# HandBrake/HandBrake

Hardware: AMD Instinct MI355X
Metric: filtered frames/sec, 1080p YUV420p NLMeans+decomb chain (higher is better)
Workload: dtype u8 (f32 NLMeans weights, 16-bit fixed-point scaler as zimg, sharpen mix = the reference's f64 expression, as one f32 multiply where init proves that equal); 1 GPU; BASELINE configs[3]: decomb(31, EEDI2 bob) -> nlmeans medium -> cropscale lanczos 1920x1080 -> 3840x2160 -> lapsharp, 1080i YUV420P 8-bit in, inputs resident in HBM; input=1920x1080, output=3840x2160, streams_per_gpu=1, content=interlaced, stream_frames=48, stage_streams=2, parallelism=1 GPU(s) x 1 independent stream(s), device=AMD Radeon Graphics (gfx950:sramecc+:xnack-, 256 CUs)

## Files before the change

handbrake_amd/csrc/eedi2.hip:

```cpp
#include "eedi2_common.h"
#include "eedi2_vote.h"
#include "eedi2_dense.h"
#include "eedi2_engine.h"
#include "eedi2_mask_cells.h"
#include "eedi2_corner.h"

#include <atomic>
#include <algorithm>

namespace {

constexpr int PEAK = 255, NEUTRAL = 128;
constexpr int EEDI_MAX_FIELDS = EEDI_MAX_BATCH;
constexpr size_t GUARD = 32768;

__constant__ uint8_t c_limlut[33] = { 6, 6, 7, 7, 8, 8, 9, 9, 9, 10, 10, 11, 11, 12, 12, 12, 12, 12, 12, 12,
                                      12, 12, 12, 12, 12, 12, 12, 12, 12, 12, 12, 255, 255 };

constexpr int LIM_N = 33, LIM_PAD = 40;
__device__ __forceinline__ void lim_fill(uint8_t *tab, int tid)
{
    if (tid < LIM_N) tab[tid] = c_limlut[tid];
}

struct P3
{
    uint8_t *a[3];
    uint8_t *b[3];
    uint8_t *c[3];
    uint8_t *d[3];
    uint8_t *e[3];
    uint8_t *f[3];
    uint8_t *g[3];
    int pitch[3], width[3], height[3];
    size_t   fstride;
    uint32_t tffbits;
    const uint32_t *pflags;
    uint32_t pepoch;
};

struct PL { uint8_t *a, *b, *c, *d, *e, *f, *g; };
__device__ __forceinline__ PL plane_ptrs(const P3 &P, int pl, size_t off)
{
    PL q = { P.a[pl] + off, P.b[pl] + off, P.c[pl] + off, P.d[pl], P.e[pl] + off, P.f[pl] + off, P.g[pl] + off };
    if (q.d) q.d += off;
    return q;
}
#define FIELD_PLANE(P)                                                      \
    const int fld = (int)blockIdx.z / 3, pl = (int)blockIdx.z - 3 * fld;    \
    const int tff = (int)(((P).tffbits >> fld) & 1u);                       \
    const PL Q = plane_ptrs((P), pl, (size_t)fld * (P).fstride);            \
     \
     \
    const bool maskless = (P).pflags[blockIdx.z] != (P).pepoch;             \
    (void)tff; (void)maskless

__device__ __forceinline__ int hbhip_align_up_dev(int v, int a) { return (v + a - 1) / a * a; }

__device__ __forceinline__ int wave_list_slots(int *counter, unsigned n)
{
    const uint64_t b0 = __ballot(n & 1u), b1 = __ballot(n & 2u), b2 = __ballot(n & 4u);
    const int total = __popcll(b0) + 2 * __popcll(b1) + 4 * __popcll(b2);
    auto below = [](uint64_t m) { return (int)__builtin_amdgcn_mbcnt_hi((uint32_t)(m >> 32), __builtin_amdgcn_mbcnt_lo((uint32_t)m, 0u)); };
    int base = 0;
    if (total)
    {
        if ((threadIdx.x & 63) == 0) base = atomicAdd(counter, total);
        base = __builtin_amdgcn_readfirstlane(base);
    }
    return base + below(b0) + 2 * below(b1) + 4 * below(b2);
}

__device__ __forceinline__ int sad3(const uint8_t *a, int ai, const uint8_t *b, int bi)
{
    return iabs((int)a[ai - 1] - (int)b[bi - 1]) + iabs((int)a[ai] - (int)b[bi]) + iabs((int)a[ai + 1] - (int)b[bi + 1]);
}

constexpr int ABSENT = 1000;

__device__ __forceinline__ int mid9(int &v0, int &v1, int &v2, int &v3, int &v4, int &v5, int &v6, int &v7, int &v8, int n)
{
    cswap(v0, v3); cswap(v1, v7); cswap(v2, v5); cswap(v4, v8);
    cswap(v0, v7); cswap(v2, v4); cswap(v3, v8); cswap(v5, v6);
    cswap(v0, v2); cswap(v1, v3); cswap(v4, v5); cswap(v7, v8);
// ... 693 lines not shown
            act |= (uint32_t)a << j;
            inactive |= (up[j] | dn[j]) & ((2u << maxdt) - 1u);
        }
        if (__any(act != 0))
        {
            const uint32_t *tr = &s_tri[0][b];
            if (__all(inactive == 0))
                calc_dir_dense_vote<RD, false, RD, 0>(tr, maxdt, up, dn, act, nt13, nt19, &s_out[0][lx]);
            else
            {
                constexpr int RH = RD >= 8 ? RD / 2 : RD;
                calc_dir_dense_vote<RH, true, RD, 0>(tr, maxdt, up, dn, act, nt13, nt19, &s_out[0][lx]);
                if constexpr (RH < RD) calc_dir_dense_vote<RD - RH, true, RD, RH>(tr, maxdt, up, dn, act, nt13, nt19, &s_out[0][lx]);
            }
#ifdef HBHIP_DEV_STATS
            if (lane == 0) { CD_STAT(8, 1); CD_STAT(9, __all(inactive == 0)); }
#endif
        }
        __syncthreads();
    }
    else if (count)
    {
        for (int p = tid; p < count; p += CD_W)
        {
            const uint32_t id = s_list[p];
            const int j = (int)(id >> 8), lx = (int)(id & 255u), y = y0 + j, px = x0 + lx, b = lx + CD_HALO - 1;
            const int startu = max(-px + 1, -maxdt), stopu = min(width - 2 - px, maxdt);
            uint64_t pass = 0;
            if (stopu >= startu)
            {
                const int nb = stopu - startu + 1;
                pass = (nb >= 64 ? ~0ull : ((1ull << nb) - 1ull)) << (startu + maxdt);
                if (y != 1)          pass &= calc_dir_window(s_bits[j], b - maxdt, lenmask);
                if (y != height - 2) pass &= __brevll(calc_dir_window(s_bits[j + 2], b - maxdt, lenmask)) >> (64 - len);
            }
#ifdef HBHIP_DEV_STATS
            {
                int n = __popcll(pass), mx = n, sm = n, ln = 1;
                for (int o = 32; o; o >>= 1) { mx = max(mx, __shfl_xor(mx, o)); sm += __shfl_xor(sm, o); ln += __shfl_xor(ln, o); }
                const uint64_t act = __ballot(1);
                if (lane == __ffsll((unsigned long long)act) - 1) { CD_STAT(3, 1); CD_STAT(4, sm); CD_STAT(5, mx); CD_STAT(6, ln); }
            }
#endif
            const uint32_t *tr = &s_tri[j][b];
            int out;
            if (len <= 32)
                out = edge ? calc_dir_search<true, uint32_t>(tr, (uint32_t)pass, maxdt, y == 1, y == height - 2, nt13, nt19)
                           : calc_dir_search<false, uint32_t>(tr, (uint32_t)pass, maxdt, false, false, nt13, nt19);
            else
                out = edge ? calc_dir_search<true, uint64_t>(tr, pass, maxdt, y == 1, y == height - 2, nt13, nt19)
                           : calc_dir_search<false, uint64_t>(tr, pass, maxdt, false, false, nt13, nt19);
            s_out[j][lx] = (uint8_t)out;
        }
        __syncthreads();
    }
#pragma unroll
    for (int jr = 0; jr < R; jr += CD_W / 64)
    {
        const int j = jr + (tid >> 6), y = y0 + j, xb = x0 + 4 * lane;
        if (j < R && y < height && xb < pitch)
            *reinterpret_cast<uint32_t *>(Q.c + (size_t)y * pitch + xb) = pad_bytes(reinterpret_cast<const uint32_t *>(&s_out[j][0])[lane], xb, width, padv);
    }
}


__device__ __forceinline__ int dir_map_px(int u0, int u1, int u2, int c0, int c1, int c2, int n0, int n1, int n2,
                                          bool up_ok, bool dn_ok, int expand, const uint8_t *limlut)
{
    const bool h0 = up_ok && u0 != PEAK, h1 = up_ok && u1 != PEAK, h2 = up_ok && u2 != PEAK;
    const bool h3 = c0 != PEAK, h4 = !expand && c1 != PEAK, h5 = c2 != PEAK;
    const bool h6 = dn_ok && n0 != PEAK, h7 = dn_ok && n1 != PEAK, h8 = dn_ok && n2 != PEAK;
    const int u = h0 + h1 + h2 + h3 + h4 + h5 + h6 + h7 + h8;
    if (u < (expand ? 5 : 4)) return expand ? c1 : PEAK;
    int v0 = h0 ? u0 : ABSENT, v1 = h1 ? u1 : ABSENT, v2 = h2 ? u2 : ABSENT;
    int v3 = h3 ? c0 : ABSENT, v4 = h4 ? c1 : ABSENT, v5 = h5 ? c2 : ABSENT;
    int v6 = h6 ? n0 : ABSENT, v7 = h7 ? n1 : ABSENT, v8 = h8 ? n2 : ABSENT;
    int s0 = v0, s1 = v1, s2 = v2, s3 = v3, s4 = v4, s5 = v5, s6 = v6, s7 = v7, s8 = v8;
    const int mid = mid9(s0, s1, s2, s3, s4, s5, s6, s7, s8, u);
    const int lim = limlut[iabs(mid - NEUTRAL) >> 2];
    int sum = 0, count = 0;
    vote1(v0, mid, lim, sum, count); vote1(v1, mid, lim, sum, count); vote1(v2, mid, lim, sum, count);
    vote1(v3, mid, lim, sum, count); vote1(v4, mid, lim, sum, count); vote1(v5, mid, lim, sum, count);
    vote1(v6, mid, lim, sum, count); vote1(v7, mid, lim, sum, count); vote1(v8, mid, lim, sum, count);
    const int val = vote_avg(sum + mid, count + 1);
    if (expand) return count >= 5 ? (val & 0xff) : c1;
    if (count < 4 || (count < 5 && c1 == PEAK)) return PEAK;
    return val & 0xff;
}

__device__ __forceinline__ uint32_t ff_bytes(uint32_t v)
{
    return (((v & 0x7f7f7f7fu) + 0x01010101u) & v) & 0x80808080u;
}

constexpr uint32_t PK_ABSENT_HI = 0x7f00u;
__device__ __forceinline__ u16x2 limlut2(u16x2 i)
{
    const u16x2 g = pk_lt(pk1(7), i);
    const u16x2 l = __builtin_elementwise_min((u16x2)(((i - g) >> 1) + pk1(6)), pk1(12));
    const u16x2 big = pk_lt(pk1(30), i) * pk1(255);
    return __builtin_elementwise_max(l, big);
}
#define PK_BYTES(hi, lo, a, b) __builtin_amdgcn_perm((hi), (lo), 0x0c000c00u | ((uint32_t)(b) << 16) | (uint32_t)(a))

template <int K>
__device__ __forceinline__ uint32_t dir_map_pair(const Win12 &wu, const Win12 &wc, const Win12 &wd, int expand)
{
    u16x2 v[9];
    {
        const Win12 *rows[3] = { &wu, &wc, &wd };
#pragma unroll
        for (int r = 0; r < 3; r++)
        {
            const uint32_t w0 = rows[r]->w0, w1 = rows[r]->w1, w2 = rows[r]->w2;
            if (K == 0)
            {
                v[3 * r + 0] = pk(PK_BYTES(w1, w0, 3, 4));
                v[3 * r + 1] = pk(PK_BYTES(w1, w0, 4, 5));
                v[3 * r + 2] = pk(PK_BYTES(w1, w0, 5, 6));
            }
            else
            {
                v[3 * r + 0] = pk(PK_BYTES(w1, w0, 5, 6));
                v[3 * r + 1] = pk(PK_BYTES(w1, w0, 6, 7));
                v[3 * r + 2] = pk(PK_BYTES(w2, w1, 3, 4));
            }
        }
    }
    const u16x2 c1 = v[4];
    u16x2 a[9];
    uint32_t absent = 0;
#pragma unroll
    for (int i = 0; i < 9; i++)
    {
        a[i] = (u16x2)((v[i] + pk1(1)) >> 8);
        absent += un(a[i]);
        v[i] = v[i] + a[i] * pk1(PK_ABSENT_HI);
    }
    u16x2 s0 = v[0], s1 = v[1], s2 = v[2], s3 = v[3], s4 = v[4], s5 = v[5], s6 = v[6], s7 = v[7], s8 = v[8];
    cswap2(s0, s3); cswap2(s1, s7); cswap2(s2, s5); cswap2(s4, s8);
    cswap2(s0, s7); cswap2(s2, s4); cswap2(s3, s8); cswap2(s5, s6);
    cswap2(s0, s2); cswap2(s1, s3); cswap2(s4, s5); cswap2(s7, s8);
    cswap2(s1, s4); cswap2(s3, s6); cswap2(s5, s7);
    cswap2(s0, s1); cswap2(s2, s4); cswap2(s3, s5); cswap2(s6, s8);
    cswap2(s2, s3); cswap2(s4, s5); cswap2(s6, s7);
    cswap2(s1, s2); cswap2(s3, s4); cswap2(s5, s6);
    const u16x2 ab = pk(absent), one = pk1(1), zero = pk1(0);
    const uint32_t m5 = un(zero - pk_lt(pk1(3), ab));
    const uint32_t m7 = un(zero - pk_lt(one, ab));
    const uint32_t modd = un((ab & one) - one);
#define PK_SEL(m, x, y) (((m) & (x)) | (~(m) & (y)))
    const uint32_t hi = PK_SEL(m5, un(s2), PK_SEL(m7, un(s3), un(s4)));
    const uint32_t lo = PK_SEL(m5, un(s1), PK_SEL(m7, un(s2), un(s3)));
    const u16x2 mid = pk(PK_SEL(modd, hi, un((u16x2)((pk(lo) + pk(hi) + one) >> 1))));
    const i16x2 t = __builtin_bit_cast(i16x2, (u16x2)(mid - pk1(NEUTRAL)));
    const u16x2 lim1 = limlut2(__builtin_bit_cast(u16x2, __builtin_elementwise_max(t, (i16x2)(-t))) >> 2) + one;
    u16x2 sum = zero, cnt = zero;
#pragma unroll
    for (int i = 0; i < 9; i++)
    {
        const u16x2 d = __builtin_elementwise_max(v[i], mid) - __builtin_elementwise_min(v[i], mid);
        const u16x2 in = pk_lt(d, lim1);
        cnt += in;
        sum += in * v[i];
    }
    const uint32_t sm = un((u16x2)(sum + mid)), ct = un(cnt);
    uint32_t out = 0;
#pragma unroll
    for (int h = 0; h < 2; h++)
    {
        const int n = 9 - (int)((absent >> (16 * h)) & 0xffffu);
        const int count = n >= 4 ? (int)((ct >> (16 * h)) & 0xffffu) : 0;
        const int val = vote_avg((int)((sm >> (16 * h)) & 0xffffu), count + 1) & 0xff;
        const int c = (int)((un(c1) >> (16 * h)) & 0xffu);
        int res;
        if (expand) res = count >= 5 ? val : c;
        else        res = (count < 4 || (count < 5 && c == PEAK)) ? PEAK : val;
        out |= (uint32_t)res << (16 * h);
    }
#undef PK_SEL
    return out;
}

__global__ __launch_bounds__(256) void k_dir_map4(P3 P, int step, int expand)
{
    FIELD_PLANE(P);
    const int x = 4 * (blockIdx.x * blockDim.x + threadIdx.x);
    const int r = blockIdx.y * blockDim.y + threadIdx.y;
    const int pitch = P.pitch[pl], width = P.width[pl], height = P.height[pl];
    const int y0 = step == 1 ? 1 : 2 - tff;
    const int y = step == 1 ? r : 2 * r + (y0 & 1);
    if (x >= width) return;
    if (maskless)
    {
        const int ya = step == 1 ? r : 2 * r, nrows = step == 1 ? 1 : 2;
        const int out[4] = { PEAK, PEAK, PEAK, PEAK };
        for (int i = 0; i < nrows && ya + i < height; i++)
        {
            const size_t at = (size_t)(ya + i) * pitch + x;
            st4(Q.c + at, out, x, width);
            if (Q.d) st4(Q.d + at, out, x, width);
        }
        return;
    }
    const int yc = 2 * r + 1 - (y0 & 1);
    const bool copy = step != 1 && yc < height;
    uint32_t vcopy = 0;
    if (copy) vcopy = *reinterpret_cast<const uint32_t *>(Q.b + (size_t)yc * pitch + x);
    auto put_copy = [&]() {
        if (!copy) return;
        int out[4] = { (int)(vcopy & 0xff), (int)((vcopy >> 8) & 0xff), (int)((vcopy >> 16) & 0xff), (int)(vcopy >> 24) };
        st4(Q.c + (size_t)yc * pitch + x, out, x, width);
        if (Q.d) st4(Q.d + (size_t)yc * pitch + x, out, x, width);
    };
    if (y >= height) { put_copy(); return; }
    const uint8_t *dc = Q.b + (size_t)y * pitch + x;
    uint8_t *o = Q.c + (size_t)y * pitch + x;
    const bool row_ok = step == 1 ? (y >= 1 && y < height - 1) : (y >= y0 && y < height - 1);
    if (!row_ok)
    {
        const uint32_t v = *reinterpret_cast<const uint32_t *>(dc);
        int out[4] = { (int)(v & 0xff), (int)((v >> 8) & 0xff), (int)((v >> 16) & 0xff), (int)(v >> 24) };
        st4(o, out, x, width);
        if (Q.d) st4(Q.d + (size_t)y * pitch + x, out, x, width);
        put_copy();
        return;
    }
    const uint32_t own = *reinterpret_cast<const uint32_t *>(dc);
    const uint8_t *mk = Q.a + (size_t)y * pitch + x;
    const uint32_t m0 = *reinterpret_cast<const uint32_t *>(step == 1 ? mk : mk - (ptrdiff_t)pitch);
    const uint32_t m1 = step == 1 ? 0u : *reinterpret_cast<const uint32_t *>(mk + pitch);
    const bool up_ok = step == 1 || y > 1, dn_ok = step == 1 || y < height - 2;
    uint32_t work = ((ff_bytes(m0) | ff_bytes(m1)) >> 7) & bytes_in(x, 1, width - 1);
    if (expand) work &= ff_bytes(own) >> 7;
    uint32_t res = own;
    if (work)
    {
        asm volatile("" ::: "memory");
        const Win12 wc = ldwin(dc), wu = ldwin(dc - (ptrdiff_t)step * pitch), wd = ldwin(dc + (ptrdiff_t)step * pitch);
        const Win12 none = { 0xffffffffu, 0xffffffffu, 0xffffffffu };
        const Win12 eu = up_ok ? wu : none, ed = dn_ok ? wd : none;
        const uint32_t p01 = dir_map_pair<0>(eu, wc, ed, expand), p23 = dir_map_pair<2>(eu, wc, ed, expand);
        const uint32_t votes = __builtin_amdgcn_perm(p23, p01, 0x06040200u);
        const uint32_t sel = work * 255u;
        res = (res & ~sel) | (votes & sel);
    }
    int out[4] = { (int)(res & 0xff), (int)((res >> 8) & 0xff), (int)((res >> 16) & 0xff), (int)(res >> 24) };
    st4(o, out, x, width);
    if (Q.d)
    {
        int in[4] = { (int)(own & 0xff), (int)((own >> 8) & 0xff), (int)((own >> 16) & 0xff), (int)(own >> 24) };
        st4(Q.d + (size_t)y * pitch + x, in, x, width);
    }
    put_copy();
}

__device__ __forceinline__ uint32_t live3(const Win12 &w, uint32_t &centre)
{
    const uint32_t n0 = (~ff_bytes(w.w0) >> 7) & 0x01010101u, n1 = (~ff_bytes(w.w1) >> 7) & 0x01010101u, n2 = (~ff_bytes(w.w2) >> 7) & 0x01010101u;
    centre = n1;
    return __builtin_amdgcn_alignbyte(n1, n0, 3) + n1 + __builtin_amdgcn_alignbyte(n2, n1, 1);
}

#ifndef DC_THREAD_ROWS
#define DC_THREAD_ROWS 4
#endif
constexpr int DC_R = DC_THREAD_ROWS, DC_ROWS = 4 * DC_R;
__global__ __launch_bounds__(256) void k_dir_map_c(P3 P, int step, int expand, int post)
{
    __shared__ __attribute__((aligned(16))) uint8_t s_out[DC_ROWS][256];
    __shared__ uint16_t s_list[DC_ROWS * 256];
    __shared__ int s_count;
    __shared__ uint8_t s_lim[LIM_PAD];
    FIELD_PLANE(P);
    const int y0 = step == 1 ? 1 : 2 - tff;
    const int rb = blockIdx.y * DC_ROWS;
    const int bx0 = 4 * (blockIdx.x * 64), x = bx0 + 4 * threadIdx.x;
    const int yb = step == 1 ? rb : 2 * rb + (y0 & 1);
    const int pitch = P.pitch[pl], width = P.width[pl], height = P.height[pl];
    if (bx0 >= width || (step == 1 ? rb : 2 * rb) >= height) return;
    if (maskless)
    {
        if (x < width)
        {
            const int out[4] = { PEAK, PEAK, PEAK, PEAK };
#pragma unroll
            for (int h = 0; h < DC_R; h++)
            {
                const int r = rb + (int)threadIdx.y + 4 * h, ya = step == 1 ? r : 2 * r, nrows = step == 1 ? 1 : 2;
                for (int i = 0; i < nrows && ya + i < height; i++)
                {
                    const size_t at = (size_t)(ya + i) * pitch + x;
                    st4(Q.c + at, out, x, width);
                    if (Q.d) st4(Q.d + at, out, x, width);
                }
            }
        }
        return;
    }
    const int tid = threadIdx.y * 64 + threadIdx.x;
    if (tid == 0) s_count = 0;
    lim_fill(s_lim, tid);
    __syncthreads();
    uint32_t vcopy[DC_R], own[DC_R], m0[DC_R], m1[DC_R], cand[DC_R];
#pragma unroll
    for (int h = 0; h < DC_R; h++)
    {
        const int lr = (int)threadIdx.y + 4 * h, r = rb + lr, y = step == 1 ? r : 2 * r + (y0 & 1);
        const int yc = 2 * r + 1 - (y0 & 1);
        vcopy[h] = 0; own[h] = 0; m0[h] = 0; m1[h] = 0;
        if (step != 1 && x < width && yc < height) vcopy[h] = *reinterpret_cast<const uint32_t *>(Q.b + (size_t)yc * pitch + x);
        const bool inside = x < width && y < height;
        const bool row_ok = step == 1 ? (y >= 1 && y < height - 1) : (y >= y0 && y < height - 1);
        if (inside)
        {
            own[h] = *reinterpret_cast<const uint32_t *>(Q.b + (size_t)y * pitch + x);
            if (row_ok)
            {
                const uint8_t *mk = Q.a + (size_t)y * pitch + x;
                m0[h] = *reinterpret_cast<const uint32_t *>(step == 1 ? mk : mk - (ptrdiff_t)pitch);
                if (step != 1) m1[h] = *reinterpret_cast<const uint32_t *>(mk + pitch);
            }
        }
    }
    Win12 wc[DC_R], wu[DC_R], wd[DC_R];
#pragma unroll
    for (int h = 0; h < DC_R; h++)
// ... 119 lines not shown
    {
        const Win12 none = { 0xffffffffu, 0xffffffffu, 0xffffffffu };
        const Win12 wc = { s_f[lr + 1][tx], own, s_f[lr + 1][tx + 2] };
        const Win12 wu = up_ok ? Win12{ s_f[lr][tx], s_f[lr][tx + 1], s_f[lr][tx + 2] } : none;
        const Win12 wd = dn_ok ? Win12{ s_f[lr + 2][tx], s_f[lr + 2][tx + 1], s_f[lr + 2][tx + 2] } : none;
        uint32_t nc, nu, nd;
        const uint32_t s3c = live3(wc, nc), s3u = live3(wu, nu), s3d = live3(wd, nd);
        const uint32_t u = s3c - nc + s3u + s3d;
        const uint32_t enough = ((u + (uint32_t)(0x80 - 5) * 0x01010101u) >> 7) & 0x01010101u;
        const uint32_t sortpx = cand & enough;
        if (sortpx)
        {
            int at = atomicAdd(s_count, __popc(sortpx));
#pragma unroll
            for (int k = 0; k < 4; k++)
                if ((sortpx >> (8 * k)) & 1u) s_list[at++] = (uint16_t)((lr << 8) | (4 * tx + k));
        }
        (void)nu; (void)nd;
    }
    *reinterpret_cast<uint32_t *>(&s_out[lr][4 * tx]) = own;
}

template <int STEP, bool POST>
__global__ __launch_bounds__(256) void k_dir_map_fe(P3 P, uint32_t padv)
{
    __shared__ uint32_t s_f[FE_R + 2][FE_LW];
    __shared__ __attribute__((aligned(16))) uint8_t s_out[FE_R][256];
    __shared__ uint16_t s_list[FE_R * 256];
    __shared__ int s_count;
    __shared__ uint8_t s_lim[LIM_PAD];
    FIELD_PLANE(P);
    const int y0 = STEP == 1 ? 1 : 2 - tff, par = STEP == 1 ? 0 : (y0 & 1);
    const int rb = blockIdx.y * FE_R;
    const int bx0 = 256 * blockIdx.x, x = bx0 + 4 * threadIdx.x;
    const int pitch = P.pitch[pl], width = P.width[pl], height = P.height[pl];
    if (bx0 >= pitch || STEP * rb >= height) return;
    auto row_ok = [&](int y) { return STEP == 1 ? (y >= 1 && y < height - 1) : (y >= y0 && y < height - 1); };
    if (maskless)
    {
        if (x < pitch)
            for (int lr = threadIdx.y; lr < FE_R; lr += 4)
#pragma unroll
                for (int i = 0; i < STEP; i++)
                    if (STEP * (rb + lr) + i < height)
                    {
                        const size_t at = (size_t)(STEP * (rb + lr) + i) * pitch + x;
                        *reinterpret_cast<uint32_t *>(Q.c + at) = pad_bytes(0xffffffffu, x, width, padv);
                        if (POST && x < width) { const int out[4] = { PEAK, PEAK, PEAK, PEAK }; st4(Q.d + at, out, x, width); }
                    }
        return;
    }
    const int tid = threadIdx.y * 64 + threadIdx.x;
    if (tid == 0) s_count = 0;
    lim_fill(s_lim, tid);
    constexpr int NCOPY = STEP == 1 ? 1 : (FE_R + 3) / 4;
    uint32_t vcopy[NCOPY];
    if (STEP != 1)
#pragma unroll
        for (int h = 0; h < NCOPY; h++)
        {
            const int lr = threadIdx.y + 4 * h, yc = 2 * (rb + lr) + 1 - par;
            vcopy[h] = (lr < FE_R && yc < height && x < width) ? *reinterpret_cast<const uint32_t *>(Q.b + (size_t)yc * pitch + x) : 0u;
        }
    auto filtered = [&](int r, int xx, auto side) -> uint32_t {
        constexpr int SIDE = decltype(side)::value;
        const int y = STEP * r + par;
        if (r < 0 || y >= height || xx < 0 || xx >= width) return 0u;
        const uint8_t *dc = Q.b + (size_t)y * pitch + xx;
        const uint32_t own = *reinterpret_cast<const uint32_t *>(dc);
        if (!row_ok(y)) return own;
        const uint8_t *mk = Q.a + (size_t)y * pitch + xx;
        const uint32_t m0 = *reinterpret_cast<const uint32_t *>(STEP == 1 ? mk : mk - (ptrdiff_t)pitch);
        const uint32_t m1 = STEP == 1 ? 0u : *reinterpret_cast<const uint32_t *>(mk + pitch);
        uint32_t work = ((ff_bytes(m0) | ff_bytes(m1)) >> 7) & bytes_in(xx, 1, width - 1);
        if (SIDE < 0) work &= 0xff000000u;
        if (SIDE > 0) work &= 0x000000ffu;
        uint32_t res = own;
        if (work)
        {
            asm volatile("" ::: "memory");
            const bool up_ok = STEP == 1 || y > 1, dn_ok = STEP == 1 || y < height - 2;
            const Win12 none = { 0xffffffffu, 0xffffffffu, 0xffffffffu };
            const Win12 wc = ldwin(dc), wu = up_ok ? ldwin(dc - (ptrdiff_t)STEP * pitch) : none, wd = dn_ok ? ldwin(dc + (ptrdiff_t)STEP * pitch) : none;
            const uint32_t p01 = SIDE < 0 ? 0u : dir_map_pair<0>(wu, wc, wd, 0), p23 = SIDE > 0 ? 0u : dir_map_pair<2>(wu, wc, wd, 0);
            const uint32_t votes = __builtin_amdgcn_perm(p23, p01, 0x06040200u);
            const uint32_t sel = work * 255u;
            res = (res & ~sel) | (votes & sel);
        }
        return res;
    };
    for (int lr = threadIdx.y; lr < FE_R + 2; lr += 4) s_f[lr][threadIdx.x + 1] = filtered(rb - 1 + lr, x, std::integral_constant<int, 0>());
    static_assert(FE_R + 2 <= 64, "a lane per ring row");
    if (threadIdx.y == 0 && (int)threadIdx.x < FE_R + 2) s_f[threadIdx.x][0] = filtered(rb - 1 + (int)threadIdx.x, bx0 - 4, std::integral_constant<int, -1>());
    if (threadIdx.y == 1 && (int)threadIdx.x < FE_R + 2) s_f[threadIdx.x][65] = filtered(rb - 1 + (int)threadIdx.x, bx0 + 256, std::integral_constant<int, 1>());
    __syncthreads();
    for (int lr = threadIdx.y; lr < FE_R; lr += 4)
    {
        const int y = STEP * (rb + lr) + par;
        if (x >= width || y >= height) continue;
        uint32_t cand = 0;
        if (row_ok(y))
        {
            const uint8_t *mk = Q.a + (size_t)y * pitch + x;
            const uint32_t m0 = *reinterpret_cast<const uint32_t *>(STEP == 1 ? mk : mk - (ptrdiff_t)pitch);
            const uint32_t m1 = STEP == 1 ? 0u : *reinterpret_cast<const uint32_t *>(mk + pitch);
            cand = ((ff_bytes(m0) | ff_bytes(m1)) >> 7) & bytes_in(x, 1, width - 1);
        }
        fe_expand_row(s_f, lr, threadIdx.x, cand, STEP == 1 || y > 1, STEP == 1 || y < height - 2, s_out, s_list, &s_count);
    }
    __syncthreads();
    const int count = s_count;
    for (int i = tid; i < count; i += 256)
    {
        const int e = s_list[i], ly = e >> 8, lx = e & 255;
        const int y = STEP * (rb + ly) + par;
        const uint8_t *c = reinterpret_cast<const uint8_t *>(&s_f[ly + 1][1]) + lx;
        const uint8_t *up = c - 4 * FE_LW, *dn = c + 4 * FE_LW;
        s_out[ly][lx] = (uint8_t)dir_map_px(up[-1], up[0], up[1], c[-1], c[0], c[1], dn[-1], dn[0], dn[1],
                                            STEP == 1 || y > 1, STEP == 1 || y < height - 2, 1, s_lim);
    }
    __syncthreads();
#pragma unroll
    for (int h = 0; h < (FE_R + 3) / 4; h++)
    {
        const int lr = threadIdx.y + 4 * h, y = STEP * (rb + lr) + par;
        if (lr >= FE_R || x >= pitch) continue;
        auto put_d = [&](int yy, uint32_t v) {
            if (x >= width) return;
            uint8_t *o = Q.d + (size_t)yy * pitch + x;
            if (x + 3 < width) *reinterpret_cast<uint32_t *>(o) = v;
            else for (int k = 0; k < 4 && x + k < width; k++) o[k] = (uint8_t)(v >> (8 * k));
        };
        if (y < height)
        {
            const uint32_t v = x < width ? *reinterpret_cast<const uint32_t *>(&s_out[lr][4 * threadIdx.x]) : 0u;
            *reinterpret_cast<uint32_t *>(Q.c + (size_t)y * pitch + x) = pad_bytes(v, x, width, padv);
            if (POST) put_d(y, s_f[lr + 1][threadIdx.x + 1]);
            if (POST && x < width && row_ok(y))
            {
                const size_t at = (size_t)y * pitch + x;
                const uint32_t om4 = *reinterpret_cast<const uint32_t *>(Q.b + at);
                uint8_t *d = Q.f + at;
                const uint32_t up4 = *reinterpret_cast<const uint32_t *>(d - pitch), dn4 = *reinterpret_cast<const uint32_t *>(d + pitch);
                const uint32_t cur4 = *reinterpret_cast<const uint32_t *>(d);
                int out[4];
                bool any = false;
#pragma unroll
                for (int k = 0; k < 4; k++)
                {
                    const int nm = (v >> (8 * k)) & 0xffu, om = (om4 >> (8 * k)) & 0xffu;
                    const int lim = s_lim[iabs(nm - NEUTRAL) >> 2];
                    const bool fix = iabs(nm - om) > lim && om != PEAK && om != NEUTRAL;
                    out[k] = fix ? (int)((((up4 >> (8 * k)) & 0xffu) + ((dn4 >> (8 * k)) & 0xffu) + 1) >> 1) : (int)((cur4 >> (8 * k)) & 0xffu);
                    any |= fix;
                }
                if (any) st4(d, out, x, width);
            }
        }
        if (STEP != 1)
        {
            const int yc = 2 * (rb + lr) + 1 - par;
            if (yc < height)
            {
                *reinterpret_cast<uint32_t *>(Q.c + (size_t)yc * pitch + x) = pad_bytes(vcopy[h < NCOPY ? h : 0], x, width, padv);
                if (POST) put_d(yc, vcopy[h < NCOPY ? h : 0]);
            }
        }
    }
}
// ... 1263 lines not shown
                if (g == 0) rc = enqueue_passes(at, k, lc, lc->stream, epoch[p]);
                else
                {
                    FORK_TRY(hipStreamWaitEvent(side_[g - 1], ready, 0));
                    if (herr != hipSuccess) break;
                    used[g - 1] = true;
                    rc = enqueue_passes(at, k, lc, side_[g - 1], epoch[p]);
                }
                at += k;
            }
        }
#undef FORK_TRY
        if (herr != hipSuccess || rc != HBHIP_OK)
        {
            for (int g = 0; g < MAX_SIDE; g++) if (used[g]) (void)hipStreamSynchronize(side_[g]);
            if (ahead_used) (void)hipStreamSynchronize(ahead_);
            if (herr != hipSuccess) rc = lc->fail(herr, hwhat);
        }
        else
            for (int g = 0; g < MAX_SIDE; g++)
                if (used[g])
                {
                    HBHIP_CHECK(lc, hipEventRecord(ev_join_[g], side_[g]));
                    HBHIP_CHECK(lc, hipStreamWaitEvent(lc->stream, ev_join_[g], 0));
                }
    }
    last_slot_ = start_ + n - 1;
    return rc;
}

int Eedi2Engine::enqueue_mask(int f0, int n, hbhip_ctx *lc, hipStream_t st, uint32_t *epoch_out)
{
    const EediFrame srcp = at_slot(half_[0], start_ + f0), mskp = at_slot(half_[1], start_ + f0),
                    mskp_old = at_slot(half_[1], f0 ? start_ + f0 - 1 : last_slot_);
    P3 P;
    memset(&P, 0, sizeof(P));
    MaskSrc S;
    memset(&S, 0, sizeof(S));
    for (int c = 0; c < 3; c++)
    {
        P.pitch[c] = srcp.stride[c]; P.width[c] = srcp.width[c]; P.height[c] = srcp.height[c];
        P.a[c] = srcp.plane[c]; P.b[c] = mskp_old.plane[c]; P.c[c] = mskp.plane[c];
        S.spitch[c] = src_pitch_[c];
    }
    for (int f = 0; f < n; f++) for (int c = 0; c < 3; c++) S.frame[f][c] = src_frame_[f0 + f][c];
    P.fstride = slot_bytes_;
    P.tffbits = tffbits_ >> f0;
    MaskChain C;
    { const int erc = begin_mask(lc, f0, (MF_OPT & 4) != 0, &C); if (erc != HBHIP_OK) return erc; }
    *epoch_out = C.epoch;
    const EediMaskThresholds th = mask_thresholds();
    if (n == 1)
        HBHIP_LAUNCH_ON(lc, st, "eedi2_mask_passes", k_mask_fused4, dim3((srcp.width[0] + MF::W - 1) / MF::W, (srcp.height[0] + MF::H - 1) / MF::H, 3),
                        dim3(MF::T), 0, P, S, 0, 0, th.mth, th.vth, th.lth, par_.erosion_threshold, par_.dilation_threshold, C.pflags, C.epoch);
    else
    {
        HBHIP_LAUNCH_ON(lc, st, "eedi2_mask_passes", k_mask_chain, dim3((unsigned)(C.group * n)), dim3(MF::T), 0, P, S, C, th.mth, th.vth, th.lth,
                     par_.erosion_threshold, par_.dilation_threshold);
        HBHIP_LAUNCH_ON(lc, st, "eedi2_mask_repair", k_mask_chain_repair, dim3(C.has ? 3u * (unsigned)n : 1u), dim3(MF::T), 0, P, S, C, n,
                        th.mth, th.vth, th.lth, par_.erosion_threshold, par_.dilation_threshold);
    }
    HBHIP_CHECK(lc, hipGetLastError());
    return HBHIP_OK;
}

int Eedi2Engine::enqueue_passes(int f0, int n, hbhip_ctx *lc, hipStream_t st, uint32_t epoch)
{
    const int s0 = start_ + f0;
    const uint32_t tffbits = tffbits_ >> f0;
    const EediFrame srcp = at_slot(half_[0], s0), mskp = at_slot(half_[1], s0), tmpp = at_slot(half_[2], s0),
                    dstp = at_slot(half_[3], s0);
    const EediFrame dst2p = at_slot(full_[0], s0), tmp2p2 = at_slot(full_[1], s0), msk2p = at_slot(full_[2], s0),
                    tmp2p = at_slot(full_[3], s0), dst2mp = at_slot(full_[4], s0);
    uint32_t *cand = reinterpret_cast<uint32_t *>(cand_raw_) + (size_t)s0 * (slot_bytes_ / sizeof(uint32_t));
    const dim3 blk(64, 4);
    const unsigned gz = 3u * (unsigned)n;
    auto grid4_for = [&](const EediFrame &f, bool whole_pitch) {
        const int w = whole_pitch ? f.stride[0] : f.width[0];
        return dim3(hbhip_grid_x((w + 255) / 256), (f.height[0] + 3) / 4, gz);
    };
    bool post_folded = false;
    auto dir_map = [&](const char *name, const EediFrame &f, const P3 &Pv, int step, int expand, int post = 0) {
        const int trows = step == 1 ? f.height[0] : (f.height[0] + 1) / 2;
        if (!expand) HBHIP_LAUNCH_ON(lc, st, name, k_dir_map4, dim3(hbhip_grid_x((f.width[0] + 255) / 256), (trows + 3) / 4, gz), blk, 0, Pv, step, expand);
        else
        {
            HBHIP_LAUNCH_ON(lc, st, name, k_dir_map_c, dim3(hbhip_grid_x((f.width[0] + 255) / 256), (trows + DC_ROWS - 1) / DC_ROWS, gz), blk, 0, Pv, step, expand, post);
            post_folded = post != 0;
        }
    };
    auto geom = [&](P3 &P, const EediFrame &f) {
        for (int c = 0; c < 3; c++) { P.pitch[c] = f.stride[c]; P.width[c] = f.width[c]; P.height[c] = f.height[c]; }
    };
    auto bind = [&](uint8_t *(&slot)[3], const EediFrame &f) { for (int c = 0; c < 3; c++) slot[c] = f.plane[c]; };

    P3 P;
    memset(&P, 0, sizeof(P));
    P.fstride = slot_bytes_;
    P.tffbits = tffbits;
    P.pflags = plane_flags_ + 3 * f0;
    P.pepoch = epoch;

    geom(P, srcp);
    const bool fused = par_.maximum_search_distance <= CD_HALO - 2 && hbhip_dev_int("HBHIP_EEDI2_FUSE_DIRMAP", 1) != 0;
    const uint32_t padv = fused ? 0u : 0xffffffffu;
    bind(P.a, mskp); bind(P.b, srcp); bind(P.c, fused ? dstp : tmpp);
    const int nt13 = (par_.noise_threshold * 13) & 0xff, nt19 = (par_.noise_threshold * 19) & 0xff;
    if (par_.maximum_search_distance <= CD_HALO - 2)
    {
        int dense_min = CD_W * 4 / 2;
#ifdef HBHIP_DEV
        const int rows = hbhip_dev_int("HBHIP_EEDI2_CALCDIR_ROWS", 4);
        dense_min = hbhip_dev_int("HBHIP_EEDI2_CALCDIR_DENSE_MIN", CD_W * rows / 2);
        if (rows == 8)
            HBHIP_LAUNCH_ON(lc, st, "eedi2_calc_directions", k_calc_dir_rows<8>,
                         dim3(hbhip_grid_x((srcp.stride[0] + CD_W - 1) / CD_W), (srcp.height[0] + 7) / 8, gz), dim3(CD_W), 0, P,
                         par_.maximum_search_distance, nt13, nt19, dense_min, padv);
        else if (rows == 6)
            HBHIP_LAUNCH_ON(lc, st, "eedi2_calc_directions", k_calc_dir_rows<6>,
                         dim3(hbhip_grid_x((srcp.stride[0] + CD_W - 1) / CD_W), (srcp.height[0] + 5) / 6, gz), dim3(CD_W), 0, P,
                         par_.maximum_search_distance, nt13, nt19, dense_min, padv);
        else if (rows == 2)
            HBHIP_LAUNCH_ON(lc, st, "eedi2_calc_directions", k_calc_dir_rows<2>,
                         dim3(hbhip_grid_x((srcp.stride[0] + CD_W - 1) / CD_W), (srcp.height[0] + 1) / 2, gz), dim3(CD_W), 0, P,
                         par_.maximum_search_distance, nt13, nt19, dense_min, padv);
        else
#endif
        HBHIP_LAUNCH_ON(lc, st, "eedi2_calc_directions", k_calc_dir_rows<4>,
                     dim3(hbhip_grid_x((srcp.stride[0] + CD_W - 1) / CD_W), (srcp.height[0] + 3) / 4, gz), dim3(CD_W), 0, P,
                     par_.maximum_search_distance, nt13, nt19, dense_min, padv);
    }
    else
    {
        size_t half_px = 0;
        for (int c = 0; c < 3; c++) half_px += (size_t)srcp.width[c] * srcp.height[c];
        P3 Q = P;
        Q.fstride = 0;
        for (int f = 0; f < n; f++)
        {
            for (int c = 0; c < 3; c++)
            {
                Q.a[c] = P.a[c] + (size_t)f * slot_bytes_; Q.b[c] = P.b[c] + (size_t)f * slot_bytes_; Q.c[c] = P.c[c] + (size_t)f * slot_bytes_;
            }
            Q.pflags = P.pflags + 3 * f;
            HBHIP_CHECK(lc, hipMemsetAsync(work_count_, 0, sizeof(int), st));
            HBHIP_LAUNCH_ON(lc, st, "eedi2_calc_directions_mark", k_calc_dir_mark, dim3((srcp.stride[0] + 63) / 64, (srcp.height[0] + 3) / 4, 3), blk, 0,
                         Q, work_list_, work_count_);
            HBHIP_LAUNCH_ON(lc, st, "eedi2_calc_directions_work", k_calc_dir_work, dim3((unsigned)((half_px + 255) / 256)), dim3(256), 0, Q,
                         (const uint32_t *)work_list_, (const int *)work_count_, par_.maximum_search_distance, nt13, nt19);
        }
    }
    if (fused)
    {
        bind(P.a, mskp); bind(P.b, dstp); bind(P.c, tmpp);
        HBHIP_LAUNCH_ON(lc, st, "eedi2_filter_expand_dir_map", (k_dir_map_fe<1, false>),
                        dim3(hbhip_grid_x((srcp.stride[0] + 255) / 256), (srcp.height[0] + FE_R - 1) / FE_R, gz), blk, 0, P, 0xffffffffu);
    }
    else
    {
        bind(P.a, mskp); bind(P.b, tmpp); bind(P.c, dstp);
        dir_map("eedi2_filter_dir_map", srcp, P, 1, 0);
        bind(P.a, mskp); bind(P.b, dstp); bind(P.c, tmpp);
        dir_map("eedi2_expand_dir_map", srcp, P, 1, 1);
    }
    bind(P.a, mskp); bind(P.b, tmpp); bind(P.c, dstp);
    HBHIP_LAUNCH_ON(lc, st, "eedi2_filter_map", k_filter_map, grid4_for(srcp, false), blk, 0, P);
    geom(P, dst2p);
// ... 75 lines not shown
```

Before: 9398 output frames/s.

## Share column sorts across pixel pairs in EEDI2 dir-map vote

Replaces the per-pair 9-element median sorting network with a shared quad routine. It presorts each 3-row column once, reuses the sorted columns between adjacent pixel pairs, and derives only ranks 1-4 for the median. It also uses a branch-free packed in-range test, a reciprocal-based vote average, and a vectorised limit lookup. The expand parameter is dropped from k_dir_map4 because expand launches go to k_dir_map_c. The goal is fewer ALU ops in the dominant EEDI2 direction-map kernels, at the risk of subtle bit-exactness differences in the rcp-based division and the absent/peak handling.

```diff
diff --git a/handbrake_amd/csrc/eedi2.hip b/handbrake_amd/csrc/eedi2.hip
--- a/handbrake_amd/csrc/eedi2.hip
+++ b/handbrake_amd/csrc/eedi2.hip
@@ -1,5 +1,6 @@
 #include "eedi2_common.h"
 #include "eedi2_vote.h"
+#include "eedi2_dirmap_vote.h"
 #include "eedi2_dense.h"
 #include "eedi2_engine.h"
 #include "eedi2_mask_cells.h"
@@ -859,7 +860,7 @@
     vote1(v0, mid, lim, sum, count); vote1(v1, mid, lim, sum, count); vote1(v2, mid, lim, sum, count);
     vote1(v3, mid, lim, sum, count); vote1(v4, mid, lim, sum, count); vote1(v5, mid, lim, sum, count);
     vote1(v6, mid, lim, sum, count); vote1(v7, mid, lim, sum, count); vote1(v8, mid, lim, sum, count);
-    const int val = vote_avg(sum + mid, count + 1);
+    const int val = dmv_vote_avg(sum + mid, count + 1);
     if (expand) return count >= 5 ? (val & 0xff) : c1;
     if (count < 4 || (count < 5 && c1 == PEAK)) return PEAK;
     return val & 0xff;
@@ -880,86 +881,13 @@
 }
 #define PK_BYTES(hi, lo, a, b) __builtin_amdgcn_perm((hi), (lo), 0x0c000c00u | ((uint32_t)(b) << 16) | (uint32_t)(a))
 
-template <int K>
-__device__ __forceinline__ uint32_t dir_map_pair(const Win12 &wu, const Win12 &wc, const Win12 &wd, int expand)
-{
-    u16x2 v[9];
-    {
-        const Win12 *rows[3] = { &wu, &wc, &wd };
-#pragma unroll
-        for (int r = 0; r < 3; r++)
-        {
-            const uint32_t w0 = rows[r]->w0, w1 = rows[r]->w1, w2 = rows[r]->w2;
-            if (K == 0)
-            {
-                v[3 * r + 0] = pk(PK_BYTES(w1, w0, 3, 4));
-                v[3 * r + 1] = pk(PK_BYTES(w1, w0, 4, 5));
-                v[3 * r + 2] = pk(PK_BYTES(w1, w0, 5, 6));
-            }
-            else
-            {
-                v[3 * r + 0] = pk(PK_BYTES(w1, w0, 5, 6));
-                v[3 * r + 1] = pk(PK_BYTES(w1, w0, 6, 7));
-                v[3 * r + 2] = pk(PK_BYTES(w2, w1, 3, 4));
-            }
-        }
-    }
-    const u16x2 c1 = v[4];
-    u16x2 a[9];
-    uint32_t absent = 0;
-#pragma unroll
-    for (int i = 0; i < 9; i++)
-    {
-        a[i] = (u16x2)((v[i] + pk1(1)) >> 8);
-        absent += un(a[i]);
-        v[i] = v[i] + a[i] * pk1(PK_ABSENT_HI);
-    }
-    u16x2 s0 = v[0], s1 = v[1], s2 = v[2], s3 = v[3], s4 = v[4], s5 = v[5], s6 = v[6], s7 = v[7], s8 = v[8];
-    cswap2(s0, s3); cswap2(s1, s7); cswap2(s2, s5); cswap2(s4, s8);
-    cswap2(s0, s7); cswap2(s2, s4); cswap2(s3, s8); cswap2(s5, s6);
-    cswap2(s0, s2); cswap2(s1, s3); cswap2(s4, s5); cswap2(s7, s8);
-    cswap2(s1, s4); cswap2(s3, s6); cswap2(s5, s7);
-    cswap2(s0, s1); cswap2(s2, s4); cswap2(s3, s5); cswap2(s6, s8);
-    cswap2(s2, s3); cswap2(s4, s5); cswap2(s6, s7);
-    cswap2(s1, s2); cswap2(s3, s4); cswap2(s5, s6);
-    const u16x2 ab = pk(absent), one = pk1(1), zero = pk1(0);
-    const uint32_t m5 = un(zero - pk_lt(pk1(3), ab));
-    const uint32_t m7 = un(zero - pk_lt(one, ab));
-    const uint32_t modd = un((ab & one) - one);
-#define PK_SEL(m, x, y) (((m) & (x)) | (~(m) & (y)))
-    const uint32_t hi = PK_SEL(m5, un(s2), PK_SEL(m7, un(s3), un(s4)));
-    const uint32_t lo = PK_SEL(m5, un(s1), PK_SEL(m7, un(s2), un(s3)));
-    const u16x2 mid = pk(PK_SEL(modd, hi, un((u16x2)((pk(lo) + pk(hi) + one) >> 1))));
-    const i16x2 t = __builtin_bit_cast(i16x2, (u16x2)(mid - pk1(NEUTRAL)));
-    const u16x2 lim1 = limlut2(__builtin_bit_cast(u16x2, __builtin_elementwise_max(t, (i16x2)(-t))) >> 2) + one;
-    u16x2 sum = zero, cnt = zero;
-#pragma unroll
-    for (int i = 0; i < 9; i++)
-    {
-        const u16x2 d = __builtin_elementwise_max(v[i], mid) - __builtin_elementwise_min(v[i], mid);
-        const u16x2 in = pk_lt(d, lim1);
-        cnt += in;
-        sum += in * v[i];
-    }
-    const uint32_t sm = un((u16x2)(sum + mid)), ct = un(cnt);
-    uint32_t out = 0;
-#pragma unroll
-    for (int h = 0; h < 2; h++)
-    {
-        const int n = 9 - (int)((absent >> (16 * h)) & 0xffffu);
-        const int count = n >= 4 ? (int)((ct >> (16 * h)) & 0xffffu) : 0;
-        const int val = vote_avg((int)((sm >> (16 * h)) & 0xffffu), count + 1) & 0xff;
-        const int c = (int)((un(c1) >> (16 * h)) & 0xffu);
-        int res;
-        if (expand) res = count >= 5 ? val : c;
-        else        res = (count < 4 || (count < 5 && c == PEAK)) ? PEAK : val;
-        out |= (uint32_t)res << (16 * h);
-    }
-#undef PK_SEL
-    return out;
-}
-
-__global__ __launch_bounds__(256) void k_dir_map4(P3 P, int step, int expand)
+template <int PAIRS>
+__device__ __forceinline__ uint32_t dir_map_quad(const Win12 &wu, const Win12 &wc, const Win12 &wd)
+{
+    return ::dir_map_quad<PAIRS>(wu.w0, wu.w1, wu.w2, wc.w0, wc.w1, wc.w2, wd.w0, wd.w1, wd.w2);
+}
+
+__global__ __launch_bounds__(256) void k_dir_map4(P3 P, int step)
 {
     FIELD_PLANE(P);
     const int x = 4 * (blockIdx.x * blockDim.x + threadIdx.x);
@@ -1008,8 +936,7 @@
     const uint32_t m0 = *reinterpret_cast<const uint32_t *>(step == 1 ? mk : mk - (ptrdiff_t)pitch);
     const uint32_t m1 = step == 1 ? 0u : *reinterpret_cast<const uint32_t *>(mk + pitch);
     const bool up_ok = step == 1 || y > 1, dn_ok = step == 1 || y < height - 2;
-    uint32_t work = ((ff_bytes(m0) | ff_bytes(m1)) >> 7) & bytes_in(x, 1, width - 1);
-    if (expand) work &= ff_bytes(own) >> 7;
+    const uint32_t work = ((ff_bytes(m0) | ff_bytes(m1)) >> 7) & bytes_in(x, 1, width - 1);
     uint32_t res = own;
     if (work)
     {
@@ -1017,9 +944,8 @@
         const Win12 wc = ldwin(dc), wu = ldwin(dc - (ptrdiff_t)step * pitch), wd = ldwin(dc + (ptrdiff_t)step * pitch);
         const Win12 none = { 0xffffffffu, 0xffffffffu, 0xffffffffu };
         const Win12 eu = up_ok ? wu : none, ed = dn_ok ? wd : none;
-        const uint32_t p01 = dir_map_pair<0>(eu, wc, ed, expand), p23 = dir_map_pair<2>(eu, wc, ed, expand);
-        const uint32_t votes = __builtin_amdgcn_perm(p23, p01, 0x06040200u);
-        const uint32_t sel = work * 255u;
+        const uint32_t votes = dir_map_quad<3>(eu, wc, ed);
+        const uint32_t sel = (work << 8) - work;
         res = (res & ~sel) | (votes & sel);
     }
     int out[4] = { (int)(res & 0xff), (int)((res >> 8) & 0xff), (int)((res >> 16) & 0xff), (int)(res >> 24) };
@@ -1305,9 +1231,8 @@
             const bool up_ok = STEP == 1 || y > 1, dn_ok = STEP == 1 || y < height - 2;
             const Win12 none = { 0xffffffffu, 0xffffffffu, 0xffffffffu };
             const Win12 wc = ldwin(dc), wu = up_ok ? ldwin(dc - (ptrdiff_t)STEP * pitch) : none, wd = dn_ok ? ldwin(dc + (ptrdiff_t)STEP * pitch) : none;
-            const uint32_t p01 = SIDE < 0 ? 0u : dir_map_pair<0>(wu, wc, wd, 0), p23 = SIDE > 0 ? 0u : dir_map_pair<2>(wu, wc, wd, 0);
-            const uint32_t votes = __builtin_amdgcn_perm(p23, p01, 0x06040200u);
-            const uint32_t sel = work * 255u;
+            const uint32_t votes = dir_map_quad<(SIDE < 0 ? 2 : SIDE > 0 ? 1 : 3)>(wu, wc, wd);
+            const uint32_t sel = (work << 8) - work;
             res = (res & ~sel) | (votes & sel);
         }
         return res;
@@ -2737,7 +2662,7 @@
     bool post_folded = false;
     auto dir_map = [&](const char *name, const EediFrame &f, const P3 &Pv, int step, int expand, int post = 0) {
         const int trows = step == 1 ? f.height[0] : (f.height[0] + 1) / 2;
-        if (!expand) HBHIP_LAUNCH_ON(lc, st, name, k_dir_map4, dim3(hbhip_grid_x((f.width[0] + 255) / 256), (trows + 3) / 4, gz), blk, 0, Pv, step, expand);
+        if (!expand) HBHIP_LAUNCH_ON(lc, st, name, k_dir_map4, dim3(hbhip_grid_x((f.width[0] + 255) / 256), (trows + 3) / 4, gz), blk, 0, Pv, step);
         else
         {
             HBHIP_LAUNCH_ON(lc, st, name, k_dir_map_c, dim3(hbhip_grid_x((f.width[0] + 255) / 256), (trows + DC_ROWS - 1) / DC_ROWS, gz), blk, 0, Pv, step, expand, post);
diff --git a/handbrake_amd/csrc/eedi2_dirmap_vote.h b/handbrake_amd/csrc/eedi2_dirmap_vote.h
--- /dev/null
+++ b/handbrake_amd/csrc/eedi2_dirmap_vote.h
@@ -0,0 +1,171 @@
+#pragma once
+#include <hip/hip_runtime.h>
+#include <cstdint>
+
+#define DMV_FN __host__ __device__ __forceinline__
+
+typedef uint16_t dmv_h2 __attribute__((ext_vector_type(2)));
+typedef int16_t dmv_i2 __attribute__((ext_vector_type(2)));
+DMV_FN dmv_h2 dmv_pk(uint32_t v) { return __builtin_bit_cast(dmv_h2, v); }
+DMV_FN uint32_t dmv_un(dmv_h2 v) { return __builtin_bit_cast(uint32_t, v); }
+DMV_FN dmv_h2 dmv_pk1(uint32_t both) { return dmv_pk(both * 0x00010001u); }
+DMV_FN dmv_h2 dmv_min(dmv_h2 a, dmv_h2 b) { return __builtin_elementwise_min(a, b); }
+DMV_FN dmv_h2 dmv_max(dmv_h2 a, dmv_h2 b) { return __builtin_elementwise_max(a, b); }
+DMV_FN void dmv_cswap(dmv_h2 &a, dmv_h2 &b) { const dmv_h2 lo = dmv_min(a, b), hi = dmv_max(a, b); a = lo; b = hi; }
+#if defined(__HIP_DEVICE_COMPILE__)
+#define DMV_KEEP(x) asm("" : "+v"(x))
+#define DMV_MAD24(a, b, c) (__umul24((a), (b)) + (c))
+#else
+#define DMV_KEEP(x) (void)(x)
+#define DMV_MAD24(a, b, c) (((a) & 0xffffffu) * ((b) & 0xffffffu) + (c))
+#endif
+DMV_FN uint32_t dmv_neg_mask(dmv_h2 v)
+{
+    uint32_t m = dmv_un(__builtin_bit_cast(dmv_h2, (dmv_i2)(__builtin_bit_cast(dmv_i2, v) >> 15)));
+    DMV_KEEP(m);
+    return m;
+}
+DMV_FN dmv_h2 dmv_lt(dmv_h2 a, dmv_h2 b) { return (dmv_h2)((dmv_h2)(a - b) >> 15); }
+
+DMV_FN uint32_t dmv_perm(uint32_t hi, uint32_t lo, uint32_t sel)
+{
+#if defined(__HIP_DEVICE_COMPILE__)
+    return __builtin_amdgcn_perm(hi, lo, sel);
+#else
+    const uint64_t w = ((uint64_t)hi << 32) | lo;
+    uint32_t r = 0;
+    for (int k = 0; k < 4; k++)
+    {
+        const uint32_t s = (sel >> (8 * k)) & 0xffu;
+        r |= (s < 8 ? (uint32_t)((w >> (8 * s)) & 0xffu) : s == 12 ? 0u : 0xffu) << (8 * k);
+    }
+    return r;
+#endif
+}
+#define DMV_BYTES(hi, lo, a, b) dmv_perm((hi), (lo), 0x0c000c00u | ((uint32_t)(b) << 16) | (uint32_t)(a))
+DMV_FN uint32_t dmv_between(uint32_t hi, uint32_t lo) { return (lo >> 16) | (hi << 16); }
+
+DMV_FN int dmv_vote_quot(uint32_t num, uint32_t den)
+{
+#if defined(__HIP_DEVICE_COMPILE__)
+    const float r = __builtin_amdgcn_rcpf((float)den);
+#else
+    const float r = 1.0f / (float)den;
+#endif
+    return (int)((float)num * r);
+}
+DMV_FN int dmv_vote_avg(int a, int b) { return dmv_vote_quot(4u * (uint32_t)a + 2u * (uint32_t)b + 1u, 4u * (uint32_t)b); }
+
+DMV_FN dmv_h2 dmv_lim1(dmv_h2 d)
+{
+    const dmv_h2 i = d >> 2;
+    const dmv_h2 g = dmv_min((dmv_h2)(i >> 3), dmv_pk1(1));
+    const dmv_h2 l1 = dmv_min((dmv_h2)(((i - g) >> 1) + dmv_pk1(7)), dmv_pk1(13));
+    uint32_t far = dmv_un((dmv_h2)(d + dmv_pk1(0x8000 - 124)));
+    DMV_KEEP(far);
+    return dmv_max(l1, dmv_pk((far >> 7) & 0x01000100u));
+}
+
+constexpr uint32_t DMV_ABSENT = 0x7fffu;
+
+DMV_FN void dmv_ranks1to4(dmv_h2 a0, dmv_h2 a1, dmv_h2 a2, dmv_h2 b0, dmv_h2 b1, dmv_h2 b2, dmv_h2 c0, dmv_h2 c1, dmv_h2 c2,
+                          dmv_h2 &s1, dmv_h2 &s2, dmv_h2 &s3, dmv_h2 &s4)
+{
+    dmv_cswap(a0, b0); dmv_cswap(b0, c0); dmv_cswap(a0, b0);
+    dmv_cswap(a1, b1); dmv_cswap(b1, c1); dmv_cswap(a1, b1);
+    const dmv_h2 h0 = dmv_min(dmv_min(a2, b2), c2);
+    s1 = dmv_min(b0, a1);
+    dmv_h2 x = dmv_max(b0, a1), c = c0, d = h0;
+    dmv_cswap(c, d);
+    s2 = dmv_min(x, c);
+    const dmv_h2 t = dmv_max(x, c), u = dmv_min(b1, d);
+    s3 = dmv_min(t, u);
+    s4 = dmv_max(t, u);
+}
+
+DMV_FN void dmv_pair_vote(const dmv_h2 *A, const dmv_h2 *B, const dmv_h2 *C, uint32_t absent, uint32_t &val, uint32_t &cnt)
+{
+    dmv_h2 s1, s2, s3, s4;
+    dmv_ranks1to4(A[0], A[1], A[2], B[0], B[1], B[2], C[0], C[1], C[2], s1, s2, s3, s4);
+    const dmv_h2 ab = dmv_pk(absent), one = dmv_pk1(1);
+    const uint32_t m5 = dmv_neg_mask(dmv_pk1(0x03ff) - ab), m7 = dmv_neg_mask(dmv_pk1(0x01ff) - ab);
+    const uint32_t meven = dmv_neg_mask(ab << 7);
+#define DMV_SEL(m, x, y) (((m) & (x)) | (~(m) & (y)))
+    const uint32_t hi = DMV_SEL(m5, dmv_un(s2), DMV_SEL(m7, dmv_un(s3), dmv_un(s4)));
+    const uint32_t lo = DMV_SEL(m5, dmv_un(s1), DMV_SEL(m7, dmv_un(s2), dmv_un(s3)));
+    const dmv_h2 mid = dmv_pk(DMV_SEL(meven, dmv_un((dmv_h2)((dmv_pk(lo) + dmv_pk(hi) + one) >> 1)), hi));
+#undef DMV_SEL
+    const dmv_i2 t = __builtin_bit_cast(dmv_i2, (dmv_h2)(mid - dmv_pk1(128)));
+    const dmv_h2 lim1 = dmv_lim1(__builtin_bit_cast(dmv_h2, __builtin_elementwise_max(t, (dmv_i2)(-t))));
+    const dmv_h2 above = dmv_min((dmv_h2)(mid + lim1), dmv_pk1(DMV_ABSENT));
+    uint32_t below_ = dmv_un((dmv_h2)(mid - lim1));
+    DMV_KEEP(below_);
+    const dmv_h2 below = dmv_pk(below_);
+    dmv_h2 sum = mid;
+    uint32_t n = 0;
+    const dmv_h2 *cols[3] = { A, B, C };
+#pragma unroll
+    for (int i = 0; i < 9; i++)
+    {
+        const dmv_h2 v = cols[i / 3][i % 3];
+        const uint32_t in = ((dmv_un((dmv_h2)(v - above)) & dmv_un((dmv_h2)(below - v))) >> 15) & 0x00010001u;
+        n += in;
+        sum += dmv_pk(in) * v;
+    }
+    const uint32_t num = dmv_un((dmv_h2)((sum << 2) + (dmv_pk(n) << 1) + dmv_pk1(3))), den = (n << 2) + 0x00040004u;
+    val = (uint32_t)dmv_vote_quot(num & 0xffffu, den & 0xffffu) | ((uint32_t)dmv_vote_quot(num >> 16, den >> 16) << 16);
+    cnt = n;
+}
+
+DMV_FN void dmv_unpack(const uint32_t (*w)[3], dmv_h2 *X, dmv_h2 *Y, dmv_h2 *Z, uint32_t &aX, uint32_t &aY, uint32_t &aZ)
+{
+    aX = aY = aZ = 0;
+#pragma unroll
+    for (int r = 0; r < 3; r++)
+    {
+        uint32_t v[3] = { DMV_BYTES(w[r][1], w[r][0], 3, 4), DMV_BYTES(w[r][1], w[r][0], 5, 6), DMV_BYTES(w[r][2], w[r][1], 3, 4) };
+        uint32_t *a[3] = { &aX, &aY, &aZ };
+#pragma unroll
+        for (int k = 0; k < 3; k++)
+        {
+            const uint32_t peak = (v[k] + 0x00010001u) & 0x01000100u;
+            *a[k] += peak;
+            v[k] = DMV_MAD24(peak >> 8, 0x7f00u, v[k]);
+        }
+        X[r] = dmv_pk(v[0]); Y[r] = dmv_pk(v[1]); Z[r] = dmv_pk(v[2]);
+    }
+}
+DMV_FN uint32_t dmv_pair_absent(uint32_t aL, uint32_t aR) { return aL + dmv_between(aR, aL) + aR; }
+
+template <int PAIRS>
+DMV_FN uint32_t dir_map_quad(uint32_t u0, uint32_t u1, uint32_t u2, uint32_t c0, uint32_t c1, uint32_t c2, uint32_t d0, uint32_t d1, uint32_t d2)
+{
+    const uint32_t w[3][3] = { { u0, u1, u2 }, { c0, c1, c2 }, { d0, d1, d2 } };
+    dmv_h2 X[3], Y[3], Z[3];
+    uint32_t aX, aY, aZ;
+    dmv_unpack(w, X, Y, Z, aX, aY, aZ);
+    dmv_cswap(X[0], X[1]); dmv_cswap(X[1], X[2]); dmv_cswap(X[0], X[1]);
+    dmv_cswap(Y[0], Y[1]); dmv_cswap(Y[1], Y[2]); dmv_cswap(Y[0], Y[1]);
+    dmv_cswap(Z[0], Z[1]); dmv_cswap(Z[1], Z[2]); dmv_cswap(Z[0], Z[1]);
+    uint32_t val01 = 0, val23 = 0, cnt01 = 0, cnt23 = 0;
+    if (PAIRS & 1)
+    {
+        dmv_h2 XY[3];
+#pragma unroll
+        for (int k = 0; k < 3; k++) XY[k] = dmv_pk(dmv_between(dmv_un(Y[k]), dmv_un(X[k])));
+        dmv_pair_vote(X, XY, Y, dmv_pair_absent(aX, aY), val01, cnt01);
+    }
+    if (PAIRS & 2)
+    {
+        dmv_h2 YZ[3];
+#pragma unroll
+        for (int k = 0; k < 3; k++) YZ[k] = dmv_pk(dmv_between(dmv_un(Z[k]), dmv_un(Y[k])));
+        dmv_pair_vote(Y, YZ, Z, dmv_pair_absent(aY, aZ), val23, cnt23);
+    }
+    const uint32_t vals = dmv_perm(val23, val01, 0x06040200u), cnts = dmv_perm(cnt23, cnt01, 0x06040200u);
+    const uint32_t peak_c = (((c1 & 0x7f7f7f7fu) + 0x01010101u) & c1) & 0x80808080u;
+    const uint32_t own = (~peak_c >> 7) & 0x01010101u;
+    const uint32_t k = (cnts + own + 0x7b7b7b7bu) & 0x80808080u;
+    const uint32_t keep = k | (k - (k >> 7));
+    return vals | ~keep;
+}
```

Result: faster. 9752 output frames/s (median of 6 runs) (+3.8%).
